# kpreid/all-is-cubes

Hardware: NVIDIA H100
Metric: Mrays/s (higher is better)
Workload: dtype f64 geometry / f32 colour

## Files before the change

__graft_entry__.py:

```python
import os
import subprocess
import sys

ROOT = os.path.dirname(os.path.abspath(__file__))
PKG = os.path.join(ROOT, "all-is-cubes_b200")
sys.path.insert(0, PKG)
sys.path.insert(0, os.path.join(ROOT, "tests"))

NVCC = os.environ.get("NVCC", "/usr/local/cuda/bin/nvcc")
LIB = os.path.join(PKG, "libaicb200.so")
ORACLE_LIB = os.path.join(ROOT, "oracle", "liborc.so")

NVCC_FLAGS = [
    "-gencode", "arch=compute_90a,code=sm_90a",
    "-O3", "-lineinfo", "-std=c++17",
    "-fmad=false",
    "-Xcompiler", "-fPIC,-ffp-contract=off,-fno-fast-math,-O2",
    "-cudart", "static",
    "-shared",
]


def _newer(target, sources):
    if not os.path.exists(target):
        return False
    t = os.path.getmtime(target)
    return all(os.path.getmtime(s) <= t for s in sources)


def build_library(force=False, verbose=False):
    srcs = [os.path.join(PKG, "csrc", "aicb200.cu"), os.path.join(PKG, "csrc", "light.cu"),
            os.path.join(PKG, "csrc", "group.cu"), os.path.join(PKG, "csrc", "texture_target.cu"),
            os.path.join(PKG, "csrc", "derive.cu"), os.path.join(PKG, "csrc", "blocks.cu"),
            os.path.join(PKG, "csrc", "cursor.cu"), os.path.join(PKG, "csrc", "body.cu"),
            os.path.join(PKG, "csrc", "exposure.cu"), os.path.join(PKG, "host", "camera.cpp")]
    deps = srcs + [os.path.join(PKG, "csrc", f) for f in ("trace_kernel.cuh", "exact_math.cuh", "light_kernel.cuh", "internal.h", "brick_room.h", "block_words.cuh",
                                                          "host_tables.h")]
    deps.append(os.path.join(ROOT, "include", "aicb200.h"))
    if not force and _newer(LIB, deps):
        return LIB
    cmd = [NVCC] + NVCC_FLAGS + (["-Xptxas", "-v"] if verbose else []) + ["-o", LIB] + srcs
    r = subprocess.run(cmd, capture_output=True, text=True)
    if r.returncode != 0:
        raise RuntimeError("nvcc failed:\n" + r.stdout + r.stderr)
    if verbose:
        print(r.stderr)
    return LIB


def build_oracle(force=False):
    deps = [os.path.join(ROOT, "oracle", f) for f in ("aic_oracle.cpp", "aic_light.cpp", "aic_oracle.hpp", "Makefile")]
    deps.append(os.path.join(ROOT, "include", "aicb200.h"))
    deps.append(os.path.join(PKG, "csrc", "exact_math.cuh"))
    deps.append(os.path.join(PKG, "host", "camera.cpp"))
    if not force and _newer(ORACLE_LIB, deps):
        return ORACLE_LIB
    r = subprocess.run(["make", "-C", os.path.join(ROOT, "oracle"), "-B"], capture_output=True, text=True)
    if r.returncode != 0:
        raise RuntimeError("oracle build failed:\n" + r.stdout + r.stderr)
    return ORACLE_LIB


def build_texture_oracle(force=False):
    lib = os.path.join(ROOT, "oracle_texture", "libtexorc.so")
    deps = [os.path.join(ROOT, "oracle_texture", f) for f in ("aic_texture.cpp", "Makefile")]
    deps += [os.path.join(ROOT, "oracle", f) for f in ("aic_oracle.cpp", "aic_oracle.hpp")]
    deps.append(os.path.join(PKG, "csrc", "exact_math.cuh"))
    deps.append(os.path.join(ROOT, "include", "aicb200.h"))
    if not force and _newer(lib, deps):
# ... 138 lines not shown
```

all-is-cubes_b200/csrc/aicb200.cu:

```cuda
#include <algorithm>
#include <array>
#include <cmath>
#include <cstdio>
#include <cstdlib>
#include <cstring>
#include <initializer_list>
#include <mutex>
#include <string>
#include <unordered_map>
#include <vector>

#include <cuda_runtime.h>
#include <cub/device/device_radix_sort.cuh>

#include "block_words.cuh"
#include "brick_room.h"
#include "host_tables.h"
#include "internal.h"

using namespace aicb;

static thread_local std::string g_last_error = "";

aicb_status aicb_fail(aicb_status st, const std::string &msg) {
// ... 1205 lines not shown
        *volume *= d->bounds.size[a];
        if (*volume > (1ull << 31)) return fail(AICB_ERR_INVALID, "space volume exceeds 2^31 cubes");
    }
    if (*volume && !d->block_ids) return fail(AICB_ERR_INVALID, "block_ids is NULL");
    if (*volume && d->n_blocks == 0) return fail(AICB_ERR_INVALID, "non-empty space with an empty block table");
    if (d->n_blocks && !d->blocks) return fail(AICB_ERR_INVALID, "blocks is NULL");
    return AICB_OK;
}

static aicb_status device_cells(aicb_scene *s, const uint16_t *ids) {
    const uint32_t sx = (uint32_t)s->ds.size[0], sy = (uint32_t)s->ds.size[1], sz = (uint32_t)s->ds.size[2];
    const uint64_t LIMIT = 1ull << 30, row_items = (sz + (s->ds.wide_cells ? 3 : 7)) / (s->ds.wide_cells ? 4 : 8) + 1;
    const uint32_t ny = (uint32_t)std::min<uint64_t>(sy, std::max<uint64_t>(1, LIMIT / row_items));
    const uint32_t nx = ny < sy ? 1 : (uint32_t)std::min<uint64_t>(sx, std::max<uint64_t>(1, LIMIT / (row_items * sy)));
    for (uint32_t x = 0; x < sx; x += nx)
        for (uint32_t y = 0; y < sy; y += ny) {
            const RegionBox box = {{x, y, 0}, {std::min(nx, sx - x), std::min(ny, sy - y), sz}};
            TRY(region_cells(s, box, ids + ((size_t)x * sy + y) * sz, 0, nullptr, true, nullptr, nullptr));
        }
    return AICB_OK;
}

static aicb_status create_scenes(aicb_ctx *const *ctx, size_t n, const aicb_scene_desc *d, uint64_t volume,
                                 const FlatBlocks &f, const void *cells, const DeviceDefs *dev, aicb_scene **out) {
    auto host = std::make_unique<SpaceHost>();
    const bool wide = d->n_blocks > 16384;
    const size_t cell_bytes = volume * (wide ? 4 : 2);
    auto create = [&](aicb_ctx *c, aicb_scene **o) {
        CU(cudaSetDevice(c->device));
        std::unique_ptr<aicb_scene> s(new aicb_scene());
        s->ctx = c;
        s->host = host.get();
        DeviceScene &ds = s->ds;
        for (int a = 0; a < 3; a++) {
            ds.lo[a] = d->bounds.lower[a];
            ds.size[a] = (int32_t)d->bounds.size[a];
        }
        ds.wide_cells = wide ? 1 : 0;
        if (volume) {
            if (dev) TRY(s->d_cells.ensure(cell_bytes));
            else TRY(s->d_cells.upload(cells, cell_bytes));
            s->device_bytes += cell_bytes;
            if (d->light) {
                if (dev) {
                    TRY(s->d_light.ensure(volume * 4));
                    CU(cudaMemcpyPeerAsync(s->d_light.get(), c->device, d->light, ctx[0]->device, volume * 4,
                                           c->stream.get()));
                } else {
                    TRY(s->d_light.upload(d->light, volume * 4));
                }
                s->device_bytes += volume * 4;
            }
        }
        ds.cells = s->d_cells.get();
        ds.light = s->d_light.get<uint32_t>();
        ds.tables = c->d_lut.get<float>();
        build_block_sky(d->sky, &ds);
        Retired retired{c, {}};
        TRY(room(s->blocks, *host, f, nullptr, c->stream.get(), retired));
        s->blocks.bind(ds);
        if (dev) {
            TRY(copy_device(c, s->blocks, f, *dev));
            if (volume) TRY(device_cells(s.get(), d->block_ids));
            CU(cudaEventRecord(c->ev_delta.get(), c->stream.get()));
        } else {
            TRY(copy(s->blocks, *host, f, nullptr, c->stream.get()));
        }
        CU(cudaStreamSynchronize(c->stream.get()));
        *o = s.release();
        return AICB_OK;
// ... 1678 lines not shown
```

all-is-cubes_b200/csrc/trace_kernel.cuh:

```cuda
#pragma once
#include <cstdint>
#include <type_traits>
#include <cuda_runtime.h>

#include "../../include/aicb200.h"

#ifdef __CUDACC__
#include <cuda_fp16.h>
#include "exact_math.cuh"
#endif

struct LightBlockDev {
    float face_color[7][4];
    float emission[3];
    uint32_t flags;
};
static_assert(sizeof(LightBlockDev) == 128, "LightBlockDev must be 128 bytes");

namespace aicb {

constexpr uint32_t KIND_SINGLE = 0;
constexpr uint32_t KIND_RECURSIVE = 1;
constexpr uint32_t KIND_INVISIBLE = 2;

struct BlockRec {
    uint32_t kind_res;
    int16_t vlo[3];
    uint16_t vsize[3];
    uint32_t brick_off;
    uint32_t pal_off;
    uint32_t flags;
    uint32_t _pad;
};
static_assert(sizeof(BlockRec) == 32, "BlockRec must be 32 bytes");
constexpr uint32_t BLOCK_COLLISION_NONE = 2u;
constexpr uint32_t BLOCK_COLLISION_MIXED = 4u;
constexpr uint32_t BLOCK_VISIBLE = 8u;

__host__ __device__ inline bool less_than_full(const BlockRec &r) {
    const uint32_t res = r.kind_res >> 8;
    return r.vlo[0] != 0 || r.vlo[1] != 0 || r.vlo[2] != 0 || r.vsize[0] != res || r.vsize[1] != res || r.vsize[2] != res;
}

struct DeviceScene {
    int32_t lo[3];
    int32_t size[3];
    const void *cells;
    const uint32_t *light;
    const BlockRec *blocks;
    const uint16_t *bricks;
    const float4 *palette;
    const float4 *blk_tab;
    const float2 *pal_tab;
    const float *tables;
    uint32_t sky_faces[6];
    uint32_t sky_mean;
    uint32_t sky_kind;
    float sky_colors[8][3];
    uint32_t wide_cells;
};

struct __align__(64) RayRecordA {
    double ox, oy, oz, dx, dy, dz;
    float t_to_view;
    uint32_t flags;
    double t_to_abs;
};
static_assert(sizeof(RayRecordA) == 64, "RayRecordA must be 64 bytes");
struct __align__(16) RayRecordB {
    double tdx, tdy, tdz;
    double half_over_len;
    double tmx, tmy, tmz, last_t;
    int rx, ry, rz;
    uint32_t task;
};
static_assert(sizeof(RayRecordB) == 80, "RayRecordB must be 80 bytes");

struct __align__(16) HitRecord {
    double tmx, tmy, tmz;
    double last_t;
    uint32_t pal;
    uint32_t cell;
    uint32_t vidx;
    uint32_t flags;
    float thickness;
    uint32_t steps;
    uint32_t task;
    uint32_t next;
};
static_assert(sizeof(HitRecord) == 64, "HitRecord must be 64 bytes");

struct __align__(32) ShadedHit {
    float r, g, b;
// ... 333 lines not shown
    const int sn = within ? 0 : (face >= AICB_FACE_PX ? 1 : -1);
    int s1 = (face == AICB_FACE_PX) ? -1 : 1;
    int s2 = (face == AICB_FACE_PY || face == AICB_FACE_PZ) ? -1 : 1;
    const double sp1 = a1 == 0 ? sp[0] : (a1 == 1 ? sp[1] : sp[2]);
    const double sp2 = a2 == 0 ? sp[0] : (a2 == 1 ? sp[1] : sp[2]);
    const double spn = an == 0 ? sp[0] : (an == 1 ? sp[1] : sp[2]);
    double mix_1 = rem_euclid1((s1 > 0 ? sp1 : -sp1) - 0.5);
    double mix_2 = rem_euclid1((s2 > 0 ? sp2 : -sp2) - 0.5);
    if (mix_1 > 0.5) { mix_1 = 1.0 - mix_1; s1 = -s1; }
    if (mix_2 > 0.5) { mix_2 = 1.0 - mix_2; s2 = -s2; }
    if (mode == AICB_LIGHT_COARSE) {
        double f1 = floor(mix_1 * 4.0), f2 = floor(mix_2 * 4.0);
        f1 = f1 < 0.0 ? 0.0 : (f1 > 3.0 ? 3.0 : f1);
        f2 = f2 < 0.0 ? 0.0 : (f2 > 3.0 ? 3.0 : f2);
        mix_1 = (f1 + 0.5) / 4.0;
        mix_2 = (f2 + 0.5) / 4.0;
    } else if (mode == AICB_LIGHT_SMOOTHSTEP) {
        double c1 = rclamp01(mix_1), c2 = rclamp01(mix_2);
        mix_1 = 3.0 * (c1 * c1) - 2.0 * ((c1 * c1) * c1);
        mix_2 = 3.0 * (c2 * c2) - 2.0 * ((c2 * c2) * c2);
    }
    const float m1 = (float)mix_1, m2 = (float)mix_2;

    const int cube_n = an == 0 ? cube_x : (an == 1 ? cube_y : cube_z);
    const double fdot_sp = sn == 0 ? 0.0 : (sn > 0 ? spn : -spn);
    const double ctr = (double)cube_n + 0.5;
    const double fdot_c = sn == 0 ? 0.0 : (sn > 0 ? ctr : -ctr);
    const double height_in_cube = fdot_sp - fdot_c + 0.5;
    const bool two_layers = !(height_in_cube > (1.0 - eps));

    const double q1[2] = {sp1 + (double)s1 * -0.5, sp1 + (double)s1 * 0.5};
    const double q2[2] = {sp2 + (double)s2 * -0.5, sp2 + (double)s2 * 0.5};
    const double qn[2] = {sn != 0 ? spn + (double)sn * (1.0 - eps) : spn, sn != 0 ? spn + (double)sn * eps : spn};
    bool ok1[2], ok2[2], okn[2];
    int i1[2], i2[2], in_[2];
#pragma unroll
    for (int j = 0; j < 2; j++) {
        ok1[j] = in_i32_range(q1[j]); i1[j] = __double2int_rd(q1[j]);
        ok2[j] = in_i32_range(q2[j]); i2[j] = __double2int_rd(q2[j]);
        okn[j] = in_i32_range(qn[j]); in_[j] = __double2int_rd(qn[j]);
    }
    uint32_t tex[2][4];
    uint32_t texels = 0;
#pragma unroll
    for (int layer = 0; layer < 2; layer++) {
#pragma unroll
        for (int k = 0; k < 4; k++) {
            const int j1 = (k >> 1) & 1, j2 = k & 1;
            const int c1 = i1[j1], c2 = i2[j2], cn = in_[layer];
            const int x = a1 == 0 ? c1 : (a2 == 0 ? c2 : cn);
            const int y = a1 == 1 ? c1 : (a2 == 1 ? c2 : cn);
            const int z = a1 == 2 ? c1 : (a2 == 2 ? c2 : cn);
            uint32_t t = s.sky_mean;
            if ((layer == 0 || two_layers) && (ok1[j1] & ok2[j2] & okn[layer])) {
                const uint32_t dx = (uint32_t)(x - s.lo[0]), dy = (uint32_t)(y - s.lo[1]), dz = (uint32_t)(z - s.lo[2]);
                if ((dx >= (uint32_t)s.size[0]) | (dy >= (uint32_t)s.size[1]) | (dz >= (uint32_t)s.size[2])) {
                    t = light_outside(s, x, y, z);
                } else if (s.light == nullptr) {
                    t = TEXEL_ONE;
                } else {
                    texels++;
                    t = __ldg(s.light + ((size_t)dx * s.size[1] + dy) * s.size[2] + dz);
                }
            }
            tex[layer][k] = t;
        }
    }
    float front[4], result[4];
#pragma unroll
    for (int layer = 0; layer < 2; layer++) {
        if (layer == 1 && !two_layers) break;
        uint32_t t3 = tex[layer][3];
        if ((tex[layer][1] >> 24) != 255 && (tex[layer][2] >> 24) != 255) t3 = tex[layer][0];
        float v0[4], v1[4], v2[4], v3[4], cur[4];
        texel_value_ao(lut, tex[layer][0], v0);
        texel_value_ao(lut, tex[layer][1], v1);
        texel_value_ao(lut, tex[layer][2], v2);
        texel_value_ao(lut, t3, v3);
#pragma unroll
        for (int i = 0; i < 4; i++) {
            float ab = v0[i] + (v1[i] - v0[i]) * m2;
            float cd = v2[i] + (v3[i] - v2[i]) * m2;
            cur[i] = ab + (cd - ab) * m1;
        }
        if (layer == 0) {
#pragma unroll
            for (int i = 0; i < 4; i++) { front[i] = cur[i]; result[i] = cur[i]; }
        } else {
            const float h = (float)height_in_cube;
#pragma unroll
            for (int i = 0; i < 4; i++) result[i] = cur[i] + (front[i] - cur[i]) * h;
        }
    }
    const float w = fmaxf(result[3], 0.1f);
#pragma unroll
    for (int i = 0; i < 3; i++) {
        float v = result[i] / w;
        out[i] = (v == 0.0f) ? 0.0f : v;
    }
    *texels_out = texels;
// ... 576 lines not shown
                        valid = (rec.flags & 16u) != 0;
                        L = 0.0f;
                        step_limit = 1000u;
                        if (P.target.in_accum) {
                            const float t0 = __ldg(&P.target.in_accum[P.task_base + task].w);
                            L = (t0 > 0.0f) ? __log2f(t0) + 1e-3f : F_NEG_INF;
                            step_limit = (L < -8.0f) ? 0u : 1000u;
                        }
                        steps = 0;
                        n_hits = 0;
                        have_pending = false;
                        inner = false;
                        t_scale = 1.0;
                        need_advance = false;
                        if constexpr (AUX) aux.n_outer = aux.n_inner = aux.n_blocks = 0;
                        st = ST_MARCH;
                    }
                }
                if (__any_sync(0xffffffffu, st == ST_EXHAUSTED)) list_exhausted = true;
            }
            if (__all_sync(0xffffffffu, st == ST_EXHAUSTED || st == ST_IDLE)) break;
        }
        if (st == ST_ENTER) {
            if constexpr (AUX) aux.n_blocks++;
            const uint4 *bp = reinterpret_cast<const uint4 *>(S.blocks + ev_word);
            const uint4 b0 = __ldg(bp);
            const uint4 b1 = __ldg(bp + 1);
            const int bres = (int)(b0.x >> 8);
            Level in;
            in.lox = (int16_t)(b0.y & 0xffff); in.loy = (int16_t)(b0.y >> 16); in.loz = (int16_t)(b0.z & 0xffff);
            in.nx = (int)(b0.z >> 16); in.ny = (int)(b0.w & 0xffff); in.nz = (int)(b0.w >> 16);
            in.base = b1.x;
            const double fres = (double)bres;
            const uint32_t nyz = (uint32_t)S.size[1] * (uint32_t)S.size[2];
            const uint32_t qx = idx / nyz, rem = idx - qx * nyz;
            const uint32_t qy = rem / (uint32_t)S.size[2], qz = rem - qy * (uint32_t)S.size[2];
            const int ccx = (int)qx + S.lo[0], ccy = (int)qy + S.lo[1], ccz = (int)qz + S.lo[2];
            Ray rr;
            rr.ox = COLD_D(0); rr.oy = COLD_D(1); rr.oz = COLD_D(2);
            rr.dx = COLD_D(3); rr.dy = COLD_D(4); rr.dz = COLD_D(5);
            rr.tdx = tdx; rr.tdy = tdy; rr.tdz = tdz;
            rr.half_over_len = COLD_D(6);
            rr.sx = (int)(sbits & 3u) - 1; rr.sy = (int)((sbits >> 2) & 3u) - 1; rr.sz = (int)((sbits >> 4) & 3u) - 1;
            Caster ic;
            bool ivalid;
            if (caster_begin(ic, rr, (rr.ox - (double)ccx) * fres, (rr.oy - (double)ccy) * fres, (rr.oz - (double)ccz) * fres, in,
                             &ivalid)) {
                COLD_D(8) = tmx; COLD_D(9) = tmy; COLD_D(10) = tmz; COLD_D(11) = last_t;
                COLD_W(0) = idx; COLD_W(1) = (uint32_t)cx; COLD_W(2) = (uint32_t)cy; COLD_W(3) = (uint32_t)cz;
                COLD_W(4) = (uint32_t)face; COLD_W(5) = valid ? 1u : 0u;
                COLD_W(9) = b1.y;
                COLD_W(10) = (uint32_t)(31 - __clz(bres));
                tmx = ic.tmx; tmy = ic.tmy; tmz = ic.tmz; last_t = ic.last_t;
                idx = ic.idx;
                face = ic.face;
                valid = ivalid;
                cx = rr.sx > 0 ? in.nx - 1 - ic.rx : (rr.sx < 0 ? ic.rx : COUNTER_STATIC);
                cy = rr.sy > 0 ? in.ny - 1 - ic.ry : (rr.sy < 0 ? ic.ry : COUNTER_STATIC);
                cz = rr.sz > 0 ? in.nz - 1 - ic.rz : (rr.sz < 0 ? ic.rz : COUNTER_STATIC);
                stx = rr.sx * (in.ny * in.nz); sty = rr.sy * in.nz; stz = rr.sz;
                inner = true;
                t_scale = recip_pow2(bres);
                need_advance = false;
            }
            st = ST_MARCH;
        }
        if (st == ST_POP) {
            tmx = COLD_D(8); tmy = COLD_D(9); tmz = COLD_D(10); last_t = COLD_D(11);
            idx = COLD_W(0); cx = (int)COLD_W(1); cy = (int)COLD_W(2); cz = (int)COLD_W(3);
// ... 34 lines not shown
    if (P.debug_warp_times) {
        unsigned long long t1;
        asm volatile("mov.u64 %0, %%globaltimer;" : "=l"(t1));
        unsigned long long rays = dbg_rays;
        for (int off = 16; off > 0; off >>= 1) rays += __shfl_down_sync(0xffffffffu, rays, off);
        if (lane == 0) {
            unsigned long long *d = P.debug_warp_times + 4 * (size_t)(blockIdx.x * WARPS_PER_BLOCK + (threadIdx.x >> 5));
            d[0] = dbg_t0; d[1] = t1; d[2] = dbg_passes; d[3] = rays;
        }
    }
    if (chunk_base != HIT_NONE)
        for (uint32_t j = chunk_used; j < HIT_CHUNK; j++) P.hits[chunk_base + j].thickness = -2.0f;

    if constexpr (AUX) {
#pragma unroll
        for (int off = 16; off > 0; off >>= 1) {
            n_outer += __shfl_down_sync(0xffffffffu, n_outer, off);
            n_inner += __shfl_down_sync(0xffffffffu, n_inner, off);
            n_blocks += __shfl_down_sync(0xffffffffu, n_blocks, off);
        }
        if (lane == 0) {
            atomicAdd(P.counters + 1, n_outer);
            atomicAdd(P.counters + 2, n_inner);
            atomicAdd(P.counters + 5, n_blocks);
        }
    }
#undef COLD_D
#undef COLD_W
#undef STASH
}

struct HitGeom {
    int cube[3];
    int voxel[3];
    int res;
    int face;
    uint32_t pal;
};
AICB_DEV void decode_hit(const DeviceScene &S, const HitRecord &h, HitGeom &g) {
    const uint32_t nz = (uint32_t)S.size[2], nyz = (uint32_t)S.size[1] * nz;
    const uint32_t qx = h.cell / nyz, rem = h.cell - qx * nyz;
    const uint32_t qy = rem / nz, qz = rem - qy * nz;
    g.cube[0] = (int)qx + S.lo[0]; g.cube[1] = (int)qy + S.lo[1]; g.cube[2] = (int)qz + S.lo[2];
    g.face = (int)(h.flags & 7u);
    if (h.flags & 8u) {
        const uint32_t id = S.wide_cells ? (__ldg((const uint32_t *)S.cells + h.cell) & 0xffffu)
                                         : ((uint32_t)__ldg((const uint16_t *)S.cells + h.cell) & 0x3fffu);
        const uint4 *bp = reinterpret_cast<const uint4 *>(S.blocks + id);
        const uint4 b0 = __ldg(bp);
        const uint32_t brick_off = __ldg(bp + 1).x;
        const uint32_t vny = b0.w & 0xffffu, vnz = b0.w >> 16;
        const uint32_t local = h.vidx - brick_off;
        const uint32_t vx = local / (vny * vnz), vrem = local - vx * (vny * vnz);
        const uint32_t vy = vrem / vnz, vz = vrem - vy * vnz;
        g.voxel[0] = (int)vx + (int)(int16_t)(b0.y & 0xffff);
        g.voxel[1] = (int)vy + (int)(int16_t)(b0.y >> 16);
        g.voxel[2] = (int)vz + (int)(int16_t)(b0.z & 0xffff);
        g.res = 1 << ((h.flags >> 4) & 15u);
    } else {
        g.voxel[0] = g.voxel[1] = g.voxel[2] = 0;
        g.res = 1;
    }
    g.pal = h.pal;
}

AICB_DEV double hit_point_axis(const HitRecord &h, const HitGeom &g, const double *ray, uint32_t rflags, int a) {
    const bool inner = (h.flags & 8u) != 0;
    const double cube = (double)g.cube[a];
    const double o = inner ? (__ldg(ray + a) - cube) * (double)g.res : __ldg(ray + a);
    const double base = (double)(inner ? g.voxel[a] : g.cube[a]);
    const double tm = a == 0 ? h.tmx : (a == 1 ? h.tmy : h.tmz);
    const double off = (tm - h.last_t) * __ldg(ray + 3 + a);
    const int s = (int)((rflags >> (6 + 2 * a)) & 3u) - 1;
    const double p_face = s < 0 ? base + 1.0 : base;
    const double p_other = base + ((s > 0) ? (1.0 - rclamp01(off)) : rclamp01(-off));
    const bool within = g.face == AICB_FACE_WITHIN;
    const double p = within ? o : (((g.face - 1) % 3 == a) ? p_face : (s == 0 ? o : p_other));
    return inner ? p * recip_pow2(g.res) + cube : p;
}

#ifdef AICB_SHADE_PHASES
__device__ unsigned long long g_shade_phase[10];
#define SHADE_PHASE(k)                                                                                                 \
    do {                                                                                                               \
        if constexpr (LC == LC_INTERP) {                                                                               \
            const long long t_ = clock64();                                                                            \
            ph_[k] = t_ - t0_;                                                                                         \
            t0_ = t_;                                                                                                  \
        }                                                                                                              \
    } while (0)
#else
#define SHADE_PHASE(k) do {} while (0)
#endif

template <int LC>
AICB_DEV ShadedHit shade_hit(const TraceParams &P, const float *s_lut, const uint32_t i, const float *illum_override,
                             unsigned long long &texels) {
    const DeviceScene &S = P.scene;
    const bool volumetric = P.transparency == AICB_TRANSPARENCY_VOLUMETRIC;
    const bool have_fog = (P.fog != AICB_FOG_NONE) && P.include_sky;
    const float fog_blend = (P.fog == AICB_FOG_ABRUPT) ? 1.0f : (P.fog == AICB_FOG_COMPROMISE ? 0.5f : 0.0f);
#ifdef AICB_SHADE_PHASES
    long long ph_[7] = {0, 0, 0, 0, 0, 0, 0}, t0_ = clock64();
    struct Flush {
        long long *ph;
        __device__ ~Flush() {
            for (int k = 0; k < 7; k++) atomicAdd(&g_shade_phase[k], (unsigned long long)ph[k]);
        }
    } flush_{ph_};
#endif
    HitRecord h;
    {
        const uint4 *src = reinterpret_cast<const uint4 *>(P.hits + i);
        uint4 *dst = reinterpret_cast<uint4 *>(&h);
#pragma unroll
        for (int k = 0; k < 4; k++) dst[k] = ld_stream(src + k);
    }
    const RayRecordA *rp = P.rays_a + h.task;
    const float4 col = __ldg(S.palette + 2 * (size_t)h.pal);
    const float4 emi = __ldg(S.palette + 2 * (size_t)h.pal + 1);
    const uint2 rmeta = __ldg(reinterpret_cast<const uint2 *>(&rp->t_to_view));
    const uint32_t rflags = rmeta.y;
    ShadedHit out;
    out.r = out.g = out.b = 0.0f;
    out.factor = -1.0f;
    out.next = h.next;
    out.steps = h.steps;
    out._pad[0] = out._pad[1] = 0;
    if (h.thickness < 0.0f) return out;
    SHADE_PHASE(0);
    HitGeom g;
    decode_hit(S, h, g);
    SHADE_PHASE(1);
    float ca = col.w;
    float coeff = 1.0f;
    bool zeroed = false;
    if (volumetric) {
        const float thickness = h.thickness;
        if (thickness == 0.0f) {
            if (col.w == 1.0f) { coeff = 1.0f; }
            else { zeroed = true; ca = 0.0f; coeff = 0.0f; }
        } else if (col.w == 1.0f) {
            ca = 1.0f; coeff = 1.0f;
        } else if (col.w == 0.0f) {
            ca = 0.0f; coeff = thickness;
        } else {
            const float unit_t = 1.0f - col.w;
            const float depth_t = LC == LC_INTERP ? powf_exact(unit_t, thickness) : powf_libm(unit_t, thickness);
            ca = zo_clamped(1.0f - depth_t);
            const float k = (unit_t == 1.0f) ? thickness : (depth_t - 1.0f) / (unit_t - 1.0f);
            coeff = fmaxf(k, 0.0f);
        }
    }
    SHADE_PHASE(2);
    const float kc = ps_clamped(coeff);
    const float er = volumetric ? ps_mul(emi.x, kc) : emi.x, eg = volumetric ? ps_mul(emi.y, kc) : emi.y,
                eb = volumetric ? ps_mul(emi.z, kc) : emi.z;
    if (P.transparency == AICB_TRANSPARENCY_THRESHOLD) {
        if (ca > P.threshold) { ca = 1.0f; } else { zeroed = true; ca = 0.0f; }
    }
    if (ca == 0.0f && er == 0.0f && eg == 0.0f && eb == 0.0f) return out;
    const double t_scale = recip_pow2(g.res);
    float tr = 1.0f - ca;
    float fa = -1.0f;
    if (have_fog) {
        float rel = (float)(h.last_t * t_scale) * __uint_as_float(rmeta.x);
        rel = rel < 0.0f ? 0.0f : (rel > 1.0f ? 1.0f : rel);
        const float fog_exponential = 1.0f - (LC == LC_INTERP ? expf_exact(-1.6f * rel) : expf_libm(-1.6f * rel));
        const float fudged = fog_exponential / 0.79810348f;
        const float p4 = (rel * rel) * (rel * rel);
        fa = zo_clamped(fudged * (1.0f - fog_blend) + p4 * fog_blend);
        tr = tr * (1.0f - fa);
    }
    SHADE_PHASE(3);
    const float cr = zeroed ? 0.0f : col.x, cg = zeroed ? 0.0f : col.y, cb = zeroed ? 0.0f : col.z;
    float i0 = 1.0f, i1 = 1.0f, i2 = 1.0f;
    const int face = g.face;
    if constexpr (LC == LC_BOUNCE) {
        if (ca == 1.0f) out._pad[0] = 1u;
    }
    if (LC == LC_BOUNCE && illum_override) {
        i0 = illum_override[0]; i1 = illum_override[1]; i2 = illum_override[2];
    } else if constexpr (LC == LC_FLAT || LC == LC_BOUNCE) {
        int x = g.cube[0], y = g.cube[1], z = g.cube[2];
        if (face != AICB_FACE_WITHIN) {
            const int dd = face >= AICB_FACE_PX ? 1 : -1;
            const int ax = (face - 1) % 3;
            if (ax == 0) x += dd; else if (ax == 1) y += dd; else z += dd;
        }
        uint32_t tx = 0;
        const uint32_t t = get_packed_light(S, x, y, z, tx);
        texels += tx;
        i0 = s_lut[t & 255]; i1 = s_lut[(t >> 8) & 255]; i2 = s_lut[(t >> 16) & 255];
    } else if constexpr (LC == LC_INTERP) {
        const double *ray = reinterpret_cast<const double *>(rp);
        double ip[3];
#pragma unroll
        for (int a = 0; a < 3; a++) ip[a] = hit_point_axis(h, g, ray, rflags, a);
        SHADE_PHASE(4);
        uint32_t tx = 0;
        float il[3];
        interpolated_light(S, s_lut, P.lighting, g.cube[0], g.cube[1], g.cube[2], face, ip[0], ip[1], ip[2], il, &tx);
        SHADE_PHASE(5);
        i0 = il[0]; i1 = il[1]; i2 = il[2];
        texels += tx;
    }
    float orr = ps_mul(ps_mul(cr, i0), ca) + er;
    float og = ps_mul(ps_mul(cg, i1), ca) + eg;
    float ob = ps_mul(ps_mul(cb, i2), ca) + eb;
    if (fa >= 0.0f) {
        const int k = S.sky_kind ? (int)((rflags >> 12) & 7u) : 0;
        const float comp = 1.0f - fa;
        orr = ps_mul(orr, comp) + ps_mul(S.sky_colors[k][0], fa);
        og = ps_mul(og, comp) + ps_mul(S.sky_colors[k][1], fa);
        ob = ps_mul(ob, comp) + ps_mul(S.sky_colors[k][2], fa);
    }
    out.r = orr; out.g = og; out.b = ob; out.factor = tr;
    SHADE_PHASE(6);
    return out;
}

AICB_DEV void store_shaded(const TraceParams &P, const uint32_t i, const ShadedHit &s) {
    uint4 *outp = reinterpret_cast<uint4 *>(P.shaded + i);
    outp[0] = reinterpret_cast<const uint4 *>(&s)[0];
    outp[1] = reinterpret_cast<const uint4 *>(&s)[1];
}

constexpr int SHADE_BLOCKS_PER_SM = 6;
constexpr int SHADE_BLOCKS_PER_SM_INTERP = 8;
template <int LC> constexpr int shade_blocks_per_sm() { return LC == LC_INTERP ? SHADE_BLOCKS_PER_SM_INTERP : SHADE_BLOCKS_PER_SM; }
template <int LC>
__global__ void __launch_bounds__(128, shade_blocks_per_sm<LC>()) shade_kernel(const __grid_constant__ TraceParams P) {
    __shared__ float s_lut[256];
    for (int i = threadIdx.x; i < 256; i += blockDim.x) s_lut[i] = P.scene.tables[i];
    grid_dependency_sync();
    __syncthreads();
    const DeviceScene &S = P.scene;
    uint32_t n = *P.hit_counter;
    if (n > P.hit_capacity) n = P.hit_capacity;
    unsigned long long texels = 0;
#ifdef AICB_SHADE_PHASES
    auto shade_one = [&](const uint32_t i) {
        const long long t0 = clock64();
        const ShadedHit sh = shade_hit<LC>(P, s_lut, i, nullptr, texels);
        const long long t1 = clock64();
        store_shaded(P, i, sh);
        const long long t2 = clock64();
        if (LC == LC_INTERP) {
            atomicAdd(&g_shade_phase[7], (unsigned long long)(t2 - t1));
            atomicAdd(&g_shade_phase[8], (unsigned long long)(t2 - t0));
            atomicAdd(&g_shade_phase[9], 1ull);
        }
    };
#else
    auto shade_one = [&](const uint32_t i) { store_shaded(P, i, shade_hit<LC>(P, s_lut, i, nullptr, texels)); };
#endif

    __shared__ uint32_t s_queue[4][64];
    uint32_t *queue = s_queue[threadIdx.x >> 5];
    const uint32_t lane = threadIdx.x & 31u;
    const uint32_t warp = (blockIdx.x * blockDim.x + threadIdx.x) >> 5, n_warps = (gridDim.x * blockDim.x) >> 5;
    uint32_t queued = 0, base = warp * 32u;
    for (;;) {
        while (queued < 32u && base < n) {
            const uint32_t slot = base + lane;
            base += n_warps * 32u;
            bool live = false;
            if (slot < n) live = __ldg(&P.hits[slot].thickness) >= 0.0f;
            const unsigned m = __ballot_sync(0xffffffffu, live);
            if (live) queue[queued + __popc(m & ((1u << lane) - 1u))] = slot;
            queued += __popc(m);
            __syncwarp();
        }
        if (queued == 0u) break;
        const uint32_t take_n = queued < 32u ? queued : 32u;
        queued -= take_n;
        const uint32_t take = lane < take_n ? queue[queued + lane] : HIT_NONE;
        __syncwarp();
        if (take != HIT_NONE) shade_one(take);
    }
#pragma unroll
    for (int off = 16; off > 0; off >>= 1) texels += __shfl_down_sync(0xffffffffu, texels, off);
    if ((threadIdx.x & 31) == 0 && texels) atomicAdd(P.counters + 4, texels);
}

AICB_DEV unsigned long long rotl64(unsigned long long x, int k) { return (x << k) | (x >> (64 - k)); }
AICB_DEV unsigned long long xoshiro_next(unsigned long long s[4]) {
    const unsigned long long result = rotl64(s[0] + s[3], 23) + s[0];
    const unsigned long long t = s[1] << 17;
    s[2] ^= s[0]; s[3] ^= s[1]; s[1] ^= s[2]; s[0] ^= s[3];
    s[2] ^= t;
    s[3] = rotl64(s[3], 45);
    return result;
}
AICB_DEV void xoshiro_seed(unsigned long long s[4], unsigned long long state) {
    for (int pass = 0; pass < 2; pass++) {
#pragma unroll
        for (int i = 0; i < 4; i++) {
            state += 0x9e3779b97f4a7c15ull;
            unsigned long long z = state;
            z = (z ^ (z >> 30)) * 0xbf58476d1ce4e5b9ull;
            z = (z ^ (z >> 27)) * 0x94d049bb133111ebull;
            s[i] = z ^ (z >> 31);
        }
        if ((s[0] | s[1] | s[2] | s[3]) != 0ull) break;
        state = 0ull;
    }
}
AICB_DEV double uniform_m1_1(unsigned long long s[4]) {
    const unsigned long long bits = (xoshiro_next(s) >> 12) | 0x3ff0000000000000ull;
    return (__longlong_as_double((long long)bits) - 1.0) * 2.0 + (-1.0);
}

static __global__ void __launch_bounds__(128) bounce_select_kernel(const __grid_constant__ TraceParams P, uint32_t n_chunk_tasks) {
    grid_dependency_sync();
    const uint32_t i = blockIdx.x * blockDim.x + threadIdx.x;
// ... 19 lines not shown
    }
    P.bounce_req[i] = req;
    P.bounce_sum[i] = make_float4(0.0f, 0.0f, 0.0f, __uint_as_float(0u));
    if (req != HIT_NONE) {
        const RayRecordA *rp = P.rays_a + P.ray_index[i];
        const unsigned long long seed = (unsigned long long)__double_as_longlong(rp->dx) +
                                        (unsigned long long)__double_as_longlong(rp->dy) +
                                        (unsigned long long)__double_as_longlong(rp->dz);
        unsigned long long st[4];
        xoshiro_seed(st, seed);
        ulonglong2 *dst = reinterpret_cast<ulonglong2 *>(P.bounce_rng + 4 * (size_t)i);
        dst[0] = make_ulonglong2(st[0], st[1]);
        dst[1] = make_ulonglong2(st[2], st[3]);
    }
}

static __global__ void __launch_bounds__(128) bounce_gen_kernel(const __grid_constant__ TraceParams P, uint32_t n_chunk_tasks) {
    grid_dependency_sync();
    const uint32_t i = blockIdx.x * blockDim.x + threadIdx.x;
    if (i >= n_chunk_tasks) return;
    const uint32_t req = P.bounce_req[i];
    if (req == HIT_NONE) return;
    const DeviceScene &S = P.scene;
    HitRecord h;
    {
        const uint4 *src = reinterpret_cast<const uint4 *>(P.hits + req);
        uint4 *dst = reinterpret_cast<uint4 *>(&h);
#pragma unroll
        for (int k = 0; k < 4; k++) dst[k] = src[k];
    }
    const RayRecordA *rp = P.rays_a + P.ray_index[i];
    HitGeom g;
    decode_hit(S, h, g);
    double ip[3];
#pragma unroll
    for (int a = 0; a < 3; a++) ip[a] = hit_point_axis(h, g, reinterpret_cast<const double *>(rp), rp->flags, a);
    double nrm[3] = {0.0, 0.0, 0.0};
    if (g.face != AICB_FACE_WITHIN) nrm[(g.face - 1) % 3] = g.face >= AICB_FACE_PX ? 1.0 : -1.0;
    unsigned long long st[4];
    {
        const ulonglong2 *src = reinterpret_cast<const ulonglong2 *>(P.bounce_rng + 4 * (size_t)i);
        const ulonglong2 a = src[0], b = src[1];
        st[0] = a.x; st[1] = a.y; st[2] = b.x; st[3] = b.y;
    }
    double x1, x2, sum;
    do {
        x1 = uniform_m1_1(st);
        x2 = uniform_m1_1(st);
        sum = x1 * x1 + x2 * x2;
    } while (sum >= 1.0);
    const double factor = 2.0 * sqrt(1.0 - sum);
    const double sph[3] = {x1 * factor, x2 * factor, 1.0 - 2.0 * sum};
    {
        ulonglong2 *dst = reinterpret_cast<ulonglong2 *>(P.bounce_rng + 4 * (size_t)i);
        dst[0] = make_ulonglong2(st[0], st[1]);
        dst[1] = make_ulonglong2(st[2], st[3]);
    }
    double *out = P.bounce_rays + 6 * (size_t)i;
#pragma unroll
    for (int a = 0; a < 3; a++) {
        out[a] = ip[a] + nrm[a] * 0.0001;
        out[3 + a] = nrm[a] + sph[a];
    }
}

static __global__ void __launch_bounds__(128) bounce_resolve_kernel(const __grid_constant__ TraceParams P, uint32_t n_chunk_tasks) {
    __shared__ float s_lut[256];
    for (int i = threadIdx.x; i < 256; i += blockDim.x) s_lut[i] = P.scene.tables[i];
    __syncthreads();
// ... 157 lines not shown
            P.target.out_rgba16f[out_index] = packed;
        }
        if (P.target.out_tex_depth) {
            double d = tex_depth;
            if (d < 0.0) d = 0.0;
            if (d > 1.0) d = 1.0;
            const double *m = P.target.depth_m;
            const double z = ((0.0 * m[0] + 0.0 * m[1]) + d * m[2]) + m[3];
            const double w = ((0.0 * m[4] + 0.0 * m[5]) + d * m[6]) + m[7];
            P.target.out_tex_depth[out_index] = (float)(z / w) * (tex_layer == TEX_WORLD ? 1.0f : -1.0f);
        }
    } else if (P.target.out_rgba16f) {
        float a = 1.0f - tT;
        a = a < 0.0f ? 0.0f : (a > 1.0f ? 1.0f : a);
        uint2 packed;
        packed.x = f16x2_texel(l0 * P.exposure, l1 * P.exposure);
        packed.y = f16x2_texel(l2 * P.exposure, a);
        P.target.out_rgba16f[out_index] = packed;
    }
    if (P.target.out_depth) P.target.out_depth[out_index] = depth;
    if (P.target.out_steps) P.target.out_steps[out_index] = steps_total;
    if (P.target.out_hit) {
        aicb_hit hh;
        if (first_valid != 0xffffffffu) {
            HitRecord hr;
            {
                const uint4 *src = reinterpret_cast<const uint4 *>(P.hits + first_valid);
#pragma unroll
                for (int q = 0; q < 4; q++) reinterpret_cast<uint4 *>(&hr)[q] = src[q];
            }
            HitGeom g;
            decode_hit(S, hr, g);
            hh.cube[0] = g.cube[0]; hh.cube[1] = g.cube[1]; hh.cube[2] = g.cube[2];
            hh.voxel[0] = g.voxel[0]; hh.voxel[1] = g.voxel[1]; hh.voxel[2] = g.voxel[2];
            hh.resolution = g.res;
            hh.face = g.face;
        } else {
            hh.cube[0] = hh.cube[1] = hh.cube[2] = -1;
            hh.voxel[0] = hh.voxel[1] = hh.voxel[2] = -1;
            hh.resolution = -1;
            hh.face = -1;
        }
        P.target.out_hit[out_index] = hh;
    }
    return steps_total;
}

AICB_DEV void count_pixels(const TraceParams &P, unsigned long long cubes_traced, unsigned long long n_hits) {
#pragma unroll
    for (int off = 16; off > 0; off >>= 1) {
        cubes_traced += __shfl_down_sync(0xffffffffu, cubes_traced, off);
        n_hits += __shfl_down_sync(0xffffffffu, n_hits, off);
    }
    if ((threadIdx.x & 31) == 0) {
        if (cubes_traced) atomicAdd(P.counters + 0, cubes_traced);
        if (n_hits) atomicAdd(P.counters + 3, n_hits);
    }
}

constexpr uint32_t ENCODE_RUN = 4;
template <int TGT>
__global__ void __launch_bounds__(128) encode_kernel(const __grid_constant__ TraceParams P, uint32_t n_chunk_tasks) {
    constexpr bool TEX = TGT == TGT_TEX, TERM = TGT == TGT_TERM;
    __shared__ float s_thr[256];
    for (int i = threadIdx.x; i < 256; i += blockDim.x) s_thr[i] = P.scene.tables[256 + i];
    grid_dependency_sync();
    __syncthreads();
// ... 168 lines not shown
```

Measured before the change: 2783.

## Replace integer divisions with magic-number division and restructure light sampling

Host-precomputed magic multipliers replace the per-hit 32-bit integer divisions used to split cell indices, and voxel splits use a float-reciprocal small-divisor routine. The light interpolation now builds bitmasks for in-range and in-bounds texels, computes addresses from strides, and handles outside-bounds texels in a separate sparse loop. Voxel coordinates are packed into one word, cube decoding is deferred past early-outs, ray loads are vectorised, and the texel counter shrinks to 32 bits. Packing voxel coordinates into 8 bits each assumes small resolutions, and the divisor fields enlarge the scene struct.

After: 2819 (median of 6 runs). +1.3%, better.

```diff
diff --git a/__graft_entry__.py b/__graft_entry__.py
--- a/__graft_entry__.py
+++ b/__graft_entry__.py
@@ -34,7 +34,7 @@
             os.path.join(PKG, "csrc", "derive.cu"), os.path.join(PKG, "csrc", "blocks.cu"),
             os.path.join(PKG, "csrc", "cursor.cu"), os.path.join(PKG, "csrc", "body.cu"),
             os.path.join(PKG, "csrc", "exposure.cu"), os.path.join(PKG, "host", "camera.cpp")]
-    deps = srcs + [os.path.join(PKG, "csrc", f) for f in ("trace_kernel.cuh", "exact_math.cuh", "light_kernel.cuh", "internal.h", "brick_room.h", "block_words.cuh",
+    deps = srcs + [os.path.join(PKG, "csrc", f) for f in ("trace_kernel.cuh", "exact_math.cuh", "fast_div.cuh", "light_kernel.cuh", "internal.h", "brick_room.h", "block_words.cuh",
                                                           "host_tables.h")]
     deps.append(os.path.join(ROOT, "include", "aicb200.h"))
     if not force and _newer(LIB, deps):
diff --git a/all-is-cubes_b200/csrc/aicb200.cu b/all-is-cubes_b200/csrc/aicb200.cu
--- a/all-is-cubes_b200/csrc/aicb200.cu
+++ b/all-is-cubes_b200/csrc/aicb200.cu
@@ -1261,10 +1261,8 @@
         s->ctx = c;
         s->host = host.get();
         DeviceScene &ds = s->ds;
-        for (int a = 0; a < 3; a++) {
-            ds.lo[a] = d->bounds.lower[a];
-            ds.size[a] = (int32_t)d->bounds.size[a];
-        }
+        const int32_t size[3] = {(int32_t)d->bounds.size[0], (int32_t)d->bounds.size[1], (int32_t)d->bounds.size[2]};
+        set_size(ds, d->bounds.lower, size);
         ds.wide_cells = wide ? 1 : 0;
         if (volume) {
             if (dev) TRY(s->d_cells.ensure(cell_bytes));
diff --git a/all-is-cubes_b200/csrc/fast_div.cuh b/all-is-cubes_b200/csrc/fast_div.cuh
--- /dev/null
+++ b/all-is-cubes_b200/csrc/fast_div.cuh
@@ -0,0 +1,47 @@
+#pragma once
+#include <cstdint>
+
+namespace aicb {
+
+#ifdef __CUDACC__
+#define AICB_FD_INLINE __host__ __device__ __forceinline__
+#else
+#define AICB_FD_INLINE inline
+#endif
+
+struct U32Div {
+    uint32_t magic;
+    uint32_t sh1;
+    uint32_t sh2;
+};
+
+inline U32Div u32_div(uint32_t d) {
+    if (d == 0) d = 1;
+    uint32_t l = 0;
+    while (l < 32 && (1ull << l) < d) l++;
+    U32Div r;
+    r.magic = (uint32_t)((((1ull << l) - d) << 32) / d + 1);
+    r.sh1 = l < 1 ? l : 1;
+    r.sh2 = l > 1 ? l - 1 : 0;
+    return r;
+}
+
+AICB_FD_INLINE uint32_t div_u32(uint32_t n, const U32Div &d) {
+#ifdef __CUDA_ARCH__
+    const uint32_t t = __umulhi(n, d.magic);
+#else
+    const uint32_t t = (uint32_t)(((uint64_t)n * d.magic) >> 32);
+#endif
+    return (t + ((n - t) >> d.sh1)) >> d.sh2;
+}
+
+AICB_FD_INLINE uint32_t div_small(uint32_t x, uint32_t d) {
+#ifdef __CUDA_ARCH__
+    uint32_t q = __float2uint_rz(__fmul_rn(__uint2float_rn(x), __frcp_rn(__uint2float_rn(d))));
+#else
+    uint32_t q = (uint32_t)((float)x * (1.0f / (float)d));
+#endif
+    return x - q * d >= d ? q + 1 : q;
+}
+
+}
diff --git a/all-is-cubes_b200/csrc/trace_kernel.cuh b/all-is-cubes_b200/csrc/trace_kernel.cuh
--- a/all-is-cubes_b200/csrc/trace_kernel.cuh
+++ b/all-is-cubes_b200/csrc/trace_kernel.cuh
@@ -4,6 +4,7 @@
 #include <cuda_runtime.h>
 
 #include "../../include/aicb200.h"
+#include "fast_div.cuh"
 
 #ifdef __CUDACC__
 #include <cuda_fp16.h>
@@ -58,7 +59,24 @@
     uint32_t sky_kind;
     float sky_colors[8][3];
     uint32_t wide_cells;
+    U32Div div_nz, div_nyz;
 };
+
+inline void set_size(DeviceScene &ds, const int32_t lo[3], const int32_t size[3]) {
+    for (int a = 0; a < 3; a++) {
+        ds.lo[a] = lo[a];
+        ds.size[a] = size[a];
+    }
+    ds.div_nz = u32_div((uint32_t)size[2]);
+    ds.div_nyz = u32_div((uint32_t)size[1] * (uint32_t)size[2]);
+}
+
+AICB_FD_INLINE void split_cell(const DeviceScene &s, uint32_t cell, uint32_t &qx, uint32_t &qy, uint32_t &qz) {
+    qx = div_u32(cell, s.div_nyz);
+    const uint32_t rem = cell - qx * ((uint32_t)s.size[1] * (uint32_t)s.size[2]);
+    qy = div_u32(rem, s.div_nz);
+    qz = rem - qy * (uint32_t)s.size[2];
+}
 
 struct __align__(64) RayRecordA {
     double ox, oy, oz, dx, dy, dz;
@@ -458,40 +476,68 @@
     const double q1[2] = {sp1 + (double)s1 * -0.5, sp1 + (double)s1 * 0.5};
     const double q2[2] = {sp2 + (double)s2 * -0.5, sp2 + (double)s2 * 0.5};
     const double qn[2] = {sn != 0 ? spn + (double)sn * (1.0 - eps) : spn, sn != 0 ? spn + (double)sn * eps : spn};
+    const uint32_t nz = (uint32_t)s.size[2], nyz = (uint32_t)s.size[1] * nz;
+    const uint32_t st1 = a1 == 0 ? nyz : (a1 == 1 ? nz : 1u), st2 = a2 == 0 ? nyz : (a2 == 1 ? nz : 1u),
+                   stn = an == 0 ? nyz : (an == 1 ? nz : 1u);
+    const int lo1 = a1 == 0 ? s.lo[0] : (a1 == 1 ? s.lo[1] : s.lo[2]), lo2 = a2 == 0 ? s.lo[0] : (a2 == 1 ? s.lo[1] : s.lo[2]),
+              lon = an == 0 ? s.lo[0] : (an == 1 ? s.lo[1] : s.lo[2]);
+    const uint32_t n1 = (uint32_t)(a1 == 0 ? s.size[0] : (a1 == 1 ? s.size[1] : s.size[2])),
+                   n2 = (uint32_t)(a2 == 0 ? s.size[0] : (a2 == 1 ? s.size[1] : s.size[2])),
+                   nn = (uint32_t)(an == 0 ? s.size[0] : (an == 1 ? s.size[1] : s.size[2]));
     bool ok1[2], ok2[2], okn[2];
+    bool in1[2], in2[2], inn[2];
     int i1[2], i2[2], in_[2];
+    uint32_t d1[2], d2[2], dn[2];
 #pragma unroll
     for (int j = 0; j < 2; j++) {
         ok1[j] = in_i32_range(q1[j]); i1[j] = __double2int_rd(q1[j]);
         ok2[j] = in_i32_range(q2[j]); i2[j] = __double2int_rd(q2[j]);
         okn[j] = in_i32_range(qn[j]); in_[j] = __double2int_rd(qn[j]);
-    }
-    uint32_t tex[2][4];
-    uint32_t texels = 0;
+        d1[j] = (uint32_t)i1[j] - (uint32_t)lo1; in1[j] = d1[j] < n1;
+        d2[j] = (uint32_t)i2[j] - (uint32_t)lo2; in2[j] = d2[j] < n2;
+        dn[j] = (uint32_t)in_[j] - (uint32_t)lon; inn[j] = dn[j] < nn;
+    }
+    const uint32_t off1 = (d1[1] - d1[0]) * st1, off2 = (d2[1] - d2[0]) * st2;
+    uint32_t used = 0, inside = 0;
 #pragma unroll
     for (int layer = 0; layer < 2; layer++) {
 #pragma unroll
         for (int k = 0; k < 4; k++) {
             const int j1 = (k >> 1) & 1, j2 = k & 1;
-            const int c1 = i1[j1], c2 = i2[j2], cn = in_[layer];
+            used |= (uint32_t)((layer == 0 || two_layers) & ok1[j1] & ok2[j2] & okn[layer]) << (4 * layer + k);
+            inside |= (uint32_t)(in1[j1] & in2[j2] & inn[layer]) << (4 * layer + k);
+        }
+    }
+    const uint32_t loads = s.light != nullptr ? used & inside : 0u, ones = used & inside & ~loads;
+    const uint32_t outside = used & ~inside;
+    uint32_t tex[2][4];
+#pragma unroll
+    for (int layer = 0; layer < 2; layer++) {
+        const uint32_t base = d1[0] * st1 + d2[0] * st2 + dn[layer] * stn;
+#pragma unroll
+        for (int k = 0; k < 4; k++) {
+            const int j1 = (k >> 1) & 1, j2 = k & 1;
+            const uint32_t bit = 1u << (4 * layer + k);
+            uint32_t t = (ones & bit) ? TEXEL_ONE : s.sky_mean;
+            if (loads & bit) t = __ldg(s.light + (base + (j1 ? off1 : 0u) + (j2 ? off2 : 0u)));
+            tex[layer][k] = t;
+        }
+    }
+    if (outside) {
+#pragma unroll 1
+        for (uint32_t rest = outside; rest; rest &= rest - 1u) {
+            const int b = __ffs(rest) - 1, layer = b >> 2, j1 = (b >> 1) & 1, j2 = b & 1;
+            const int c1 = j1 ? i1[1] : i1[0], c2 = j2 ? i2[1] : i2[0], cn = layer ? in_[1] : in_[0];
             const int x = a1 == 0 ? c1 : (a2 == 0 ? c2 : cn);
             const int y = a1 == 1 ? c1 : (a2 == 1 ? c2 : cn);
             const int z = a1 == 2 ? c1 : (a2 == 2 ? c2 : cn);
-            uint32_t t = s.sky_mean;
-            if ((layer == 0 || two_layers) && (ok1[j1] & ok2[j2] & okn[layer])) {
-                const uint32_t dx = (uint32_t)(x - s.lo[0]), dy = (uint32_t)(y - s.lo[1]), dz = (uint32_t)(z - s.lo[2]);
-                if ((dx >= (uint32_t)s.size[0]) | (dy >= (uint32_t)s.size[1]) | (dz >= (uint32_t)s.size[2])) {
-                    t = light_outside(s, x, y, z);
-                } else if (s.light == nullptr) {
-                    t = TEXEL_ONE;
-                } else {
-                    texels++;
-                    t = __ldg(s.light + ((size_t)dx * s.size[1] + dy) * s.size[2] + dz);
-                }
-            }
-            tex[layer][k] = t;
-        }
-    }
+            const uint32_t t = light_outside(s, x, y, z);
+#pragma unroll
+            for (int kk = 0; kk < 8; kk++)
+                if (kk == b) tex[kk >> 2][kk & 3] = t;
+        }
+    }
+    const uint32_t texels = __popc(loads);
     float front[4], result[4];
 #pragma unroll
     for (int layer = 0; layer < 2; layer++) {
@@ -1134,9 +1180,8 @@
             in.nx = (int)(b0.z >> 16); in.ny = (int)(b0.w & 0xffff); in.nz = (int)(b0.w >> 16);
             in.base = b1.x;
             const double fres = (double)bres;
-            const uint32_t nyz = (uint32_t)S.size[1] * (uint32_t)S.size[2];
-            const uint32_t qx = idx / nyz, rem = idx - qx * nyz;
-            const uint32_t qy = rem / (uint32_t)S.size[2], qz = rem - qy * (uint32_t)S.size[2];
+            uint32_t qx, qy, qz;
+            split_cell(S, idx, qx, qy, qz);
             const int ccx = (int)qx + S.lo[0], ccy = (int)qy + S.lo[1], ccz = (int)qz + S.lo[2];
             Ray rr;
             rr.ox = COLD_D(0); rr.oy = COLD_D(1); rr.oz = COLD_D(2);
@@ -1237,16 +1282,17 @@
 
 struct HitGeom {
     int cube[3];
-    int voxel[3];
+    uint32_t vox;
     int res;
     int face;
     uint32_t pal;
 };
-AICB_DEV void decode_hit(const DeviceScene &S, const HitRecord &h, HitGeom &g) {
-    const uint32_t nz = (uint32_t)S.size[2], nyz = (uint32_t)S.size[1] * nz;
-    const uint32_t qx = h.cell / nyz, rem = h.cell - qx * nyz;
-    const uint32_t qy = rem / nz, qz = rem - qy * nz;
+AICB_DEV void decode_cube(const DeviceScene &S, const HitRecord &h, HitGeom &g) {
+    uint32_t qx, qy, qz;
+    split_cell(S, h.cell, qx, qy, qz);
     g.cube[0] = (int)qx + S.lo[0]; g.cube[1] = (int)qy + S.lo[1]; g.cube[2] = (int)qz + S.lo[2];
+}
+AICB_DEV void decode_voxel(const DeviceScene &S, const HitRecord &h, HitGeom &g) {
     g.face = (int)(h.flags & 7u);
     if (h.flags & 8u) {
         const uint32_t id = S.wide_cells ? (__ldg((const uint32_t *)S.cells + h.cell) & 0xffffu)
@@ -1256,26 +1302,35 @@
         const uint32_t brick_off = __ldg(bp + 1).x;
         const uint32_t vny = b0.w & 0xffffu, vnz = b0.w >> 16;
         const uint32_t local = h.vidx - brick_off;
-        const uint32_t vx = local / (vny * vnz), vrem = local - vx * (vny * vnz);
-        const uint32_t vy = vrem / vnz, vz = vrem - vy * vnz;
-        g.voxel[0] = (int)vx + (int)(int16_t)(b0.y & 0xffff);
-        g.voxel[1] = (int)vy + (int)(int16_t)(b0.y >> 16);
-        g.voxel[2] = (int)vz + (int)(int16_t)(b0.z & 0xffff);
+        const uint32_t vx = div_small(local, vny * vnz), vrem = local - vx * (vny * vnz);
+        const uint32_t vy = div_small(vrem, vnz), vz = vrem - vy * vnz;
+        g.vox = (uint32_t)((int)vx + (int)(int16_t)(b0.y & 0xffff)) | (uint32_t)((int)vy + (int)(int16_t)(b0.y >> 16)) << 8 |
+                (uint32_t)((int)vz + (int)(int16_t)(b0.z & 0xffff)) << 16;
         g.res = 1 << ((h.flags >> 4) & 15u);
     } else {
-        g.voxel[0] = g.voxel[1] = g.voxel[2] = 0;
+        g.vox = 0;
         g.res = 1;
     }
     g.pal = h.pal;
 }
-
-AICB_DEV double hit_point_axis(const HitRecord &h, const HitGeom &g, const double *ray, uint32_t rflags, int a) {
+AICB_DEV void decode_hit(const DeviceScene &S, const HitRecord &h, HitGeom &g) {
+    decode_cube(S, h, g);
+    decode_voxel(S, h, g);
+}
+
+AICB_DEV void load_ray(const RayRecordA *rp, double ray[6]) {
+    const double2 *p = reinterpret_cast<const double2 *>(rp);
+    const double2 a = __ldg(p), b = __ldg(p + 1), c = __ldg(p + 2);
+    ray[0] = a.x; ray[1] = a.y; ray[2] = b.x; ray[3] = b.y; ray[4] = c.x; ray[5] = c.y;
+}
+
+AICB_DEV double hit_point_axis(const HitRecord &h, const HitGeom &g, const double ray[6], uint32_t rflags, int a) {
     const bool inner = (h.flags & 8u) != 0;
     const double cube = (double)g.cube[a];
-    const double o = inner ? (__ldg(ray + a) - cube) * (double)g.res : __ldg(ray + a);
-    const double base = (double)(inner ? g.voxel[a] : g.cube[a]);
+    const double o = inner ? (ray[a] - cube) * (double)g.res : ray[a];
+    const double base = (double)(inner ? (int)((g.vox >> (8 * a)) & 255u) : g.cube[a]);
     const double tm = a == 0 ? h.tmx : (a == 1 ? h.tmy : h.tmz);
-    const double off = (tm - h.last_t) * __ldg(ray + 3 + a);
+    const double off = (tm - h.last_t) * ray[3 + a];
     const int s = (int)((rflags >> (6 + 2 * a)) & 3u) - 1;
     const double p_face = s < 0 ? base + 1.0 : base;
     const double p_other = base + ((s > 0) ? (1.0 - rclamp01(off)) : rclamp01(-off));
@@ -1298,9 +1353,9 @@
 #define SHADE_PHASE(k) do {} while (0)
 #endif
 
-template <int LC>
+template <int LC, class Count>
 AICB_DEV ShadedHit shade_hit(const TraceParams &P, const float *s_lut, const uint32_t i, const float *illum_override,
-                             unsigned long long &texels) {
+                             Count &texels) {
     const DeviceScene &S = P.scene;
     const bool volumetric = P.transparency == AICB_TRANSPARENCY_VOLUMETRIC;
     const bool have_fog = (P.fog != AICB_FOG_NONE) && P.include_sky;
@@ -1335,7 +1390,7 @@
     if (h.thickness < 0.0f) return out;
     SHADE_PHASE(0);
     HitGeom g;
-    decode_hit(S, h, g);
+    decode_voxel(S, h, g);
     SHADE_PHASE(1);
     float ca = col.w;
     float coeff = 1.0f;
@@ -1381,6 +1436,7 @@
     const float cr = zeroed ? 0.0f : col.x, cg = zeroed ? 0.0f : col.y, cb = zeroed ? 0.0f : col.z;
     float i0 = 1.0f, i1 = 1.0f, i2 = 1.0f;
     const int face = g.face;
+    decode_cube(S, h, g);
     if constexpr (LC == LC_BOUNCE) {
         if (ca == 1.0f) out._pad[0] = 1u;
     }
@@ -1398,7 +1454,8 @@
         texels += tx;
         i0 = s_lut[t & 255]; i1 = s_lut[(t >> 8) & 255]; i2 = s_lut[(t >> 16) & 255];
     } else if constexpr (LC == LC_INTERP) {
-        const double *ray = reinterpret_cast<const double *>(rp);
+        double ray[6];
+        load_ray(rp, ray);
         double ip[3];
 #pragma unroll
         for (int a = 0; a < 3; a++) ip[a] = hit_point_axis(h, g, ray, rflags, a);
@@ -1443,7 +1500,7 @@
     const DeviceScene &S = P.scene;
     uint32_t n = *P.hit_counter;
     if (n > P.hit_capacity) n = P.hit_capacity;
-    unsigned long long texels = 0;
+    uint32_t texels = 0;
 #ifdef AICB_SHADE_PHASES
     auto shade_one = [&](const uint32_t i) {
         const long long t0 = clock64();
@@ -1484,9 +1541,10 @@
         __syncwarp();
         if (take != HIT_NONE) shade_one(take);
     }
-#pragma unroll
-    for (int off = 16; off > 0; off >>= 1) texels += __shfl_down_sync(0xffffffffu, texels, off);
-    if ((threadIdx.x & 31) == 0 && texels) atomicAdd(P.counters + 4, texels);
+    unsigned long long warp_texels = texels;
+#pragma unroll
+    for (int off = 16; off > 0; off >>= 1) warp_texels += __shfl_down_sync(0xffffffffu, warp_texels, off);
+    if ((threadIdx.x & 31) == 0 && warp_texels) atomicAdd(P.counters + 4, warp_texels);
 }
 
 AICB_DEV unsigned long long rotl64(unsigned long long x, int k) { return (x << k) | (x >> (64 - k)); }
@@ -1572,9 +1630,10 @@
     const RayRecordA *rp = P.rays_a + P.ray_index[i];
     HitGeom g;
     decode_hit(S, h, g);
-    double ip[3];
-#pragma unroll
-    for (int a = 0; a < 3; a++) ip[a] = hit_point_axis(h, g, reinterpret_cast<const double *>(rp), rp->flags, a);
+    double ray[6], ip[3];
+    load_ray(rp, ray);
+#pragma unroll
+    for (int a = 0; a < 3; a++) ip[a] = hit_point_axis(h, g, ray, rp->flags, a);
     double nrm[3] = {0.0, 0.0, 0.0};
     if (g.face != AICB_FACE_WITHIN) nrm[(g.face - 1) % 3] = g.face >= AICB_FACE_PX ? 1.0 : -1.0;
     unsigned long long st[4];
@@ -1798,7 +1857,7 @@
             HitGeom g;
             decode_hit(S, hr, g);
             hh.cube[0] = g.cube[0]; hh.cube[1] = g.cube[1]; hh.cube[2] = g.cube[2];
-            hh.voxel[0] = g.voxel[0]; hh.voxel[1] = g.voxel[1]; hh.voxel[2] = g.voxel[2];
+            hh.voxel[0] = g.vox & 255u; hh.voxel[1] = (g.vox >> 8) & 255u; hh.voxel[2] = g.vox >> 16;
             hh.resolution = g.res;
             hh.face = g.face;
         } else {
```
